# endiqq/Multi-Feature-ViT

Measured on AMD Instinct MI355X. Metric: images/sec (two-stream 224^2 vit_small MF-CA train step), higher is better.
Workload: dtype bf16x3 (split bf16 hi+lo operands, 3 MFMAs per product, f32 accumulate)

## Files before the change

include/mfvit.h:

```cpp
#ifndef MFVIT_H
#define MFVIT_H
#include <stddef.h>
#include <stdint.h>

#ifdef __cplusplus
extern "C" {
#endif

typedef void* mfvit_stream_t;

#define MFVIT_OK 0
#define MFVIT_EINVAL (-22)
#define MFVIT_ENOSYS (-38)
#define MFVIT_ELAUNCH (-5)

#define MFVIT_F32 0
#define MFVIT_BF16 1
#define MFVIT_BF16X3 2
#define MFVIT_F16 3
#define MFVIT_X3F16 4

int mfvit_abi_version(void);
const char* mfvit_build_info(void);

// ... 56 lines not shown
    void* scratch;
} mfvit_vit_attn_req;
size_t mfvit_vit_attn_scratch_bytes(const mfvit_vit_cfg* cfg, const mfvit_vit_attn_req* req);
int mfvit_vit_forward_attn(const mfvit_vit_cfg* cfg, const mfvit_vit_attn_req* req, const float* params, const void* shadow,
                           const float* img, void* workspace, float* features, mfvit_stream_t stream);

typedef struct mfvit_vit_rel_req {
    uint64_t blocks;
    float* maps;
    float* relevance;
    void* scratch;
} mfvit_vit_rel_req;
size_t mfvit_vit_rel_scratch_bytes(const mfvit_vit_cfg* cfg, const mfvit_vit_rel_req* req);
int mfvit_vit_backward_rel(const mfvit_vit_cfg* cfg, const mfvit_vit_rel_req* req, const float* params, const void* shadow, void* workspace,
                           const float* dfeatures, mfvit_stream_t stream);

int mfvit_gpt_forward(const mfvit_vit_cfg* cfg, const float* params, const void* shadow, const float* tokens, void* workspace, float* out,
                      mfvit_stream_t stream);
int mfvit_gpt_backward(const mfvit_vit_cfg* cfg, const float* params, const void* shadow, void* workspace, const float* dout, float* dparams,
                       float* dtokens, mfvit_stream_t stream);

int mfvit_linear_fwd(int dtype, int epilogue, const void* x, int64_t ldx, const void* w, int64_t ldw, const float* bias, void* y,
                     int64_t ldy, void* y2, int64_t ldy2, int M, int N, int K, mfvit_stream_t stream);
int mfvit_linear_dgrad_act(int dtype, const void* dy, int64_t lddy, const void* wt, int64_t ldwt, const void* act_grad, int64_t ldg,
                           void* dx, int64_t lddx, int M, int N, int K, mfvit_stream_t stream);
int mfvit_linear_wgrad(int dtype, const void* dy, int64_t lddy, const void* x, int64_t ldx, float* dw, int64_t lddw, int M, int N, int K,
                       mfvit_stream_t stream);
#define MFVIT_WGRAD_SCRATCH_FLOATS (384 * 128 * 128)
int mfvit_linear_wgrad_ws(int dtype, const void* dy, int64_t lddy, const void* x, int64_t ldx, float* dw, int64_t lddw, int M, int N,
                          int K, float* scratch, mfvit_stream_t stream);
int mfvit_linear_wgrad_pair(int dtype, const void* dy_a, int64_t lddy_a, const void* x_a, int64_t ldx_a, float* dw_a, int64_t lddw_a, float* dbias_a,
                            int Na, const void* dy_b, int64_t lddy_b, const void* x_b, int64_t ldx_b, float* dw_b, int64_t lddw_b, int Nb, int M, int K,
                            mfvit_stream_t stream);
int mfvit_linear_res_ln_fwd(int dtype, const void* a, int64_t lda, const void* w, int64_t ldw, const float* bias, const float* res,
                            int64_t ldres, float* x_out, void* y, int y_f32, const float* gamma, const float* beta, float eps,
                            float* mean, float* rstd, int M, int K, mfvit_stream_t stream);
int mfvit_linear_dgrad_ln_bwd(int dtype, const void* dy, int64_t lddy, const void* wt, int64_t ldwt, const float* x, const float* mean,
                              const float* rstd, const float* gamma, const float* dres, float* dx, void* dx_t, float* dgamma,
                              float* dbeta, float* dcol, int M, int K, mfvit_stream_t stream);
#define MFVIT_ROWP_SCRATCH_FLOATS (264 * 7 * 12 * 512)
int mfvit_linear_res_ln_fwd_ws(int dtype, const void* a, int64_t lda, const void* w, int64_t ldw, const float* bias, const float* res,
                               int64_t ldres, float* x_out, void* y, int y_f32, const float* gamma, const float* beta, float eps,
                               float* mean, float* rstd, int M, int K, float* scratch, mfvit_stream_t stream);
int mfvit_linear_dgrad_ln_bwd_ws(int dtype, const void* dy, int64_t lddy, const void* wt, int64_t ldwt, const float* x, const float* mean,
                                 const float* rstd, const float* gamma, const float* dres, float* dx, void* dx_t, float* dgamma,
                                 float* dbeta, float* dcol, int M, int K, float* scratch, mfvit_stream_t stream);
int mfvit_attention_qkv_dtype(int dtype, int T, int head_dim);
int mfvit_attention_fwd(int dtype, const void* qkv, void* out, float* lse, int B, int T, int H, int head_dim, mfvit_stream_t stream);
int mfvit_attention_bwd(int dtype, const void* qkv, const void* out, const void* dout, const float* lse, void* dqkv, float* dbias_qkv,
                        int B, int T, int H, int head_dim, mfvit_stream_t stream);
int mfvit_attention_drop_fwd(int dtype, const void* qkv, void* out, float* lse, int B, int T, int H, int head_dim, float p, uint64_t seed,
                             uint32_t site, mfvit_stream_t stream);
int mfvit_attention_drop_bwd(int dtype, const void* qkv, const void* out, const void* dout, const float* lse, void* dqkv, int B, int T, int H,
                             int head_dim, float p, uint64_t seed, uint32_t site, mfvit_stream_t stream);
int mfvit_dropout_mask(float p, uint64_t seed, uint32_t site, int64_t n, uint8_t* keep, mfvit_stream_t stream);
int mfvit_layernorm_fwd(int dtype, const float* x, void* y, int y_f32, const float* gamma, const float* beta, float eps, float* mean,
                        float* rstd, int rows, int N, mfvit_stream_t stream);
int mfvit_layernorm_bwd(int dtype, const float* dy, const float* x, const float* mean, const float* rstd, const float* gamma,
                        const float* dres, float* dx, void* dx_t, float* dgamma, float* dbeta, float* dcol, int rows, int N,
                        mfvit_stream_t stream);
int mfvit_cast_transpose(int dtype, const float* src, void* dst, void* dst_t, int R, int C, mfvit_stream_t stream);
int mfvit_head_fwd(const float* x, int64_t ldx, const float* w, const float* b, float* y, int64_t ldy, int M, int N, int K, int accumulate,
                   mfvit_stream_t stream);
int mfvit_head_bwd(const float* dy, int64_t lddy, const float* x, int64_t ldx, const float* w, float* dx, int64_t lddx, int dx_accumulate,
                   float* dw, float* db, int M, int N, int K, mfvit_stream_t stream);
int mfvit_cross_entropy(const float* logits, const int64_t* target, float* loss_mean, float* dlogits, int64_t* preds, int B, int C,
// ... 101 lines not shown
```

multi-feature-vit_amd/csrc/abi_ops.hip:

```cpp
#include "../../include/mfvit.h"
#include "kernels.h"

using namespace mfvit;

extern "C" {

int mfvit_input_transform(const uint8_t* src, const int64_t* desc, const int32_t* tables, int n, int S, int crop, const float* mean3,
                          const float* std3, float* out, mfvit_stream_t stream) {
    if (!src || !desc || !tables || !mean3 || !std3 || !out) return MFVIT_EINVAL;
    if (crop > S) return MFVIT_EINVAL;
    return input_transform(src, (const long long*)desc, tables, n, S, crop, crop, mean3, std3, out, (hipStream_t)stream);
}
int mfvit_input_transform_rect(const uint8_t* src, const int64_t* desc, const int32_t* tables, int n, int S, int out_h, int out_w,
                               const float* mean3, const float* std3, float* out, mfvit_stream_t stream) {
    if (!src || !desc || !tables || !mean3 || !std3 || !out) return MFVIT_EINVAL;
    return input_transform(src, (const long long*)desc, tables, n, S, out_h, out_w, mean3, std3, out, (hipStream_t)stream);
}
size_t mfvit_input_photometric_workspace_bytes(int n, int S) { return input_photometric_workspace_bytes(n, S); }
int mfvit_input_photometric(const uint8_t* src, const int64_t* desc, const int32_t* tables, const int32_t* photo, int n, int S, int max_radius,
                            void* workspace, const float* mean3, const float* std3, float* out, mfvit_stream_t stream) {
    if (!src || !desc || !tables || !photo || !workspace || !mean3 || !std3 || !out) return MFVIT_EINVAL;
    return input_photometric(src, (const long long*)desc, tables, photo, n, S, max_radius, workspace, mean3, std3, out, (hipStream_t)stream);
}
int mfvit_eval_counts(const float* scores, int64_t ld, const int64_t* labels, int n, int C, uint64_t* confusion, int64_t* preds,
// ... 12 lines not shown
    return gemm_nt_tile(dtype, epilogue, p, (hipStream_t)stream);
}
int mfvit_linear_dgrad_act(int dtype, const void* dy, int64_t lddy, const void* wt, int64_t ldwt, const void* act_grad, int64_t ldg,
                           void* dx, int64_t lddx, int M, int N, int K, mfvit_stream_t stream) {
    if (!dy || !wt || !act_grad || !dx) return MFVIT_EINVAL;
    GemmP p = nt(dy, lddy, wt, ldwt, M, N, K);
    p.aux = act_grad; p.ldaux = ldg; p.out0 = dx; p.ldo0 = lddx;
    return gemm_nt_tile(dtype, EPI_GELU_BWD, p, (hipStream_t)stream);
}
int mfvit_linear_wgrad(int dtype, const void* dy, int64_t lddy, const void* x, int64_t ldx, float* dw, int64_t lddw, int M, int N, int K,
                       mfvit_stream_t stream) {
    if (!dy || !x || !dw) return MFVIT_EINVAL;
    GemmP p = nt(dy, lddy, x, ldx, M, N, K);
    p.out0 = dw; p.ldo0 = lddw;
    return gemm_tn(dtype, p, (hipStream_t)stream);
}
int mfvit_linear_wgrad_ws(int dtype, const void* dy, int64_t lddy, const void* x, int64_t ldx, float* dw, int64_t lddw, int M, int N,
                          int K, float* scratch, mfvit_stream_t stream) {
    if (!dy || !x || !dw) return MFVIT_EINVAL;
    GemmP p = nt(dy, lddy, x, ldx, M, N, K);
    p.out0 = dw; p.ldo0 = lddw;
    p.cpart = scratch;
    return gemm_tn(dtype, p, (hipStream_t)stream);
}
int mfvit_linear_wgrad_pair(int dtype, const void* dy_a, int64_t lddy_a, const void* x_a, int64_t ldx_a, float* dw_a, int64_t lddw_a, float* dbias_a,
                            int Na, const void* dy_b, int64_t lddy_b, const void* x_b, int64_t ldx_b, float* dw_b, int64_t lddw_b, int Nb, int M, int K,
                            mfvit_stream_t stream) {
    if (!dy_a || !x_a || !dw_a || !dy_b || !x_b || !dw_b) return MFVIT_EINVAL;
    GemmP a = nt(dy_a, lddy_a, x_a, ldx_a, M, Na, K), b = nt(dy_b, lddy_b, x_b, ldx_b, M, Nb, K);
    a.out0 = dw_a; a.ldo0 = lddw_a; a.cs0 = dbias_a;
    b.out0 = dw_b; b.ldo0 = lddw_b;
    if (!gemm_tn_pair_supported(dtype, a, b)) return MFVIT_ENOSYS;
    return gemm_tn_glds_pair(dtype, a, b, (hipStream_t)stream);
}
int mfvit_linear_res_ln_fwd(int dtype, const void* a, int64_t lda, const void* w, int64_t ldw, const float* bias, const float* res,
                            int64_t ldres, float* x_out, void* y, int y_f32, const float* gamma, const float* beta, float eps,
                            float* mean, float* rstd, int M, int K, mfvit_stream_t stream) {
    return mfvit_linear_res_ln_fwd_ws(dtype, a, lda, w, ldw, bias, res, ldres, x_out, y, y_f32, gamma, beta, eps, mean, rstd, M, K, nullptr, stream);
}
int mfvit_linear_res_ln_fwd_ws(int dtype, const void* a, int64_t lda, const void* w, int64_t ldw, const float* bias, const float* res,
                               int64_t ldres, float* x_out, void* y, int y_f32, const float* gamma, const float* beta, float eps,
                               float* mean, float* rstd, int M, int K, float* scratch, mfvit_stream_t stream) {
    if (!a || !w || !y || !gamma || !beta || ((size_t)scratch & 15)) return MFVIT_EINVAL;
    GemmP p = nt(a, lda, w, ldw, M, 384, K);
    p.kpart = scratch;
    p.bias = bias; p.res = res; p.ldres = ldres;
    p.out0 = x_out; p.ldo0 = 384; p.out1 = y; p.ldo1 = (dtype == MFVIT_BF16X3 && !y_f32) ? 768 : 384; p.y_f32 = y_f32;
    p.gamma = gamma; p.beta = beta; p.eps = eps; p.mean = mean; p.rstd = rstd;
    return gemm_nt_row(dtype, REPI_RES_LN, p, (hipStream_t)stream);
}
int mfvit_linear_dgrad_ln_bwd(int dtype, const void* dy, int64_t lddy, const void* wt, int64_t ldwt, const float* x, const float* mean,
                              const float* rstd, const float* gamma, const float* dres, float* dx, void* dx_t, float* dgamma,
                              float* dbeta, float* dcol, int M, int K, mfvit_stream_t stream) {
    return mfvit_linear_dgrad_ln_bwd_ws(dtype, dy, lddy, wt, ldwt, x, mean, rstd, gamma, dres, dx, dx_t, dgamma, dbeta, dcol, M, K, nullptr, stream);
}
int mfvit_linear_dgrad_ln_bwd_ws(int dtype, const void* dy, int64_t lddy, const void* wt, int64_t ldwt, const float* x, const float* mean,
                                 const float* rstd, const float* gamma, const float* dres, float* dx, void* dx_t, float* dgamma,
                                 float* dbeta, float* dcol, int M, int K, float* scratch, mfvit_stream_t stream) {
    if (!dy || !wt || !x || !mean || !rstd || !gamma || !dx || ((size_t)scratch & 15)) return MFVIT_EINVAL;
    GemmP p = nt(dy, lddy, wt, ldwt, M, 384, K);
    p.kpart = scratch;
    p.aux = x; p.ldaux = 384; p.mean = (float*)mean; p.rstd = (float*)rstd; p.gamma = gamma;
    p.res = dres; p.ldres = 384;
    p.out0 = dx; p.ldo0 = 384; p.out1 = dx_t; p.ldo1 = dtype == MFVIT_BF16X3 ? 768 : 384;
    p.cs0 = dgamma; p.cs1 = dbeta; p.cs2 = dcol;
    return gemm_nt_row(dtype, REPI_LNBWD_RES, p, (hipStream_t)stream);
// ... 62 lines not shown
```

multi-feature-vit_amd/csrc/gemm.cuh:

```cuda
#pragma once
#include "common.cuh"

#include <type_traits>

namespace mfvit {

template <typename T> struct MmaTraits;
template <> struct MmaTraits<bf16> {
    typedef bf16x8 frag_t;
    static constexpr int KSTEP = 16;
    static __device__ __forceinline__ f32x16 mma(frag_t a, frag_t b, f32x16 c) {
        return __builtin_amdgcn_mfma_f32_32x32x16_bf16(a, b, c, 0, 0, 0);
    }
};
template <> struct MmaTraits<sbf16> : MmaTraits<bf16> {};
template <> struct MmaTraits<f16> {
    typedef f16x8 frag_t;
    static constexpr int KSTEP = 16;
    static __device__ __forceinline__ f32x16 mma(frag_t a, frag_t b, f32x16 c) {
        return __builtin_amdgcn_mfma_f32_32x32x16_f16(a, b, c, 0, 0, 0);
    }
};
template <> struct MmaTraits<float> {
    typedef float frag_t;
    static constexpr int KSTEP = 2;
    static __device__ __forceinline__ f32x16 mma(frag_t a, frag_t b, f32x16 c) {
        return __builtin_amdgcn_mfma_f32_32x32x2f32(a, b, c, 0, 0, 0);
    }
};

template <typename T, int R, int BKB> struct KTile;

template <typename T, int R, int BKB> struct KTile16 {
    static constexpr int CPR = BKB / 16;
// ... 120 lines not shown
            const int q = tid + i * NT, m = q / CPRW, c = q % CPRW;
            *(uint4*)(t + ((long)m * Tile::LD + c * EPC) * sizeof(T)) = reg[i];
        }
    }
};

struct GemmP {
    const void* A; long lda;
    const void* W; long ldw;
    int M, N, K;
    const float* bias;
    void* out0; long ldo0;
    void* out1; long ldo1;
    const void* aux; long ldaux;
    const float* res; long ldres;
    const void* res_t; long ldres_t;
    int res_mod, res_off;
    int orow_in, orow_out, orow_off;
    const float* gamma; const float* beta; float eps;
    float* mean; float* rstd;
    float* cs0; float* cs1; float* cs2;
    float* cpart;
    int y_f32;
    int splits;
    float* kpart;
    unsigned* kcnt;
    int rows_per_wg;
    unsigned* omax;
    int omax_rows, omax_hd;
    int nb, nbi;
    long sAo, sAi, sWo, sWi, sOo, sOi, sBo, sBi;
    DropP drop;
    int drop_tpr;
};

template <typename T> __device__ __forceinline__ void apply_batch(GemmP& p, int out_elem_bytes) {
    if (p.nb <= 1) return;
    const int z = blockIdx.z, zo = z / p.nbi, zi = z % p.nbi;
    p.A = (const T*)p.A + zo * p.sAo + zi * p.sAi;
    p.W = (const T*)p.W + zo * p.sWo + zi * p.sWi;
    p.out0 = (char*)p.out0 + (zo * p.sOo + zi * p.sOi) * out_elem_bytes;
    if (p.bias) p.bias += zo * p.sBo + zi * p.sBi;
}

__device__ __forceinline__ int out_row(const GemmP& p, int m) {
    return p.orow_in ? (m / p.orow_in) * p.orow_out + (m % p.orow_in) + p.orow_off : m;
}

__device__ __forceinline__ int acc_row(int reg, int lane) { return (reg & 3) + 8 * (reg >> 2) + 4 * (lane >> 5); }

template <typename T, int BM, int BN, int BKB, int WM, int WN> struct NtLoop {
    static constexpr int NT = WM * WN * 64;
    static constexpr int BK = BKB / (int)sizeof(T);
    static constexpr int TM = BM / WM / 32, TN = BN / WN / 32;
    typedef KTile<T, BM, BKB> TA;
    typedef KTile<T, BN, BKB> TB;
    static constexpr int STAGE_BYTES = TA::BYTES + TB::BYTES;
    static constexpr int LDS_BYTES = 2 * STAGE_BYTES;
    static constexpr bool SPLIT = is_split<T>::value;
    static constexpr bool HALF = SPLIT && BKB == 64;
    static_assert(!SPLIT || BKB == 128 || BKB == 64, "a split K tile is one 32-wide k group ([hi x 32 | lo x 32] = 128 bytes per row) or half of one");

    static __device__ __forceinline__ void compute(const char* ta, const char* tb, int wm, int wn, int lane, f32x16 (&acc)[TM][TN]) {
        if constexpr (HALF) {
            typename MmaTraits<T>::frag_t ah[TM], al[TM], bh[TN], bl[TN];
#pragma unroll
// ... 265 lines not shown
```

multi-feature-vit_amd/csrc/gemm_tn2.hip:

```cpp
#include <stdlib.h>

#include <type_traits>
#include "gemm.cuh"
#include "kernels.h"
#include "prof.h"

namespace mfvit {

namespace {

constexpr int T2_NS = 3;
constexpr int T2_NSP = 4;
constexpr int T2_TILE = 16 * 1024;
constexpr int T2_STAGE = 2 * T2_TILE;

template <typename T> struct T2Geo {
    static constexpr bool SPLIT = is_split<T>::value;
    static constexpr int TW = SPLIT ? 256 : 128;
    static constexpr int KR = SPLIT ? 32 : 64;
    static constexpr int ROWB = TW * 2;
    static constexpr int CPR = ROWB / 16;
    static constexpr int RPI = 64 / CPR;
    static constexpr int NF = TW / 2 / 32;
    static constexpr int BL = 128;
// ... 9 lines not shown
                 : "memory");
}

template <typename T> __device__ __forceinline__ typename Vec8<T>::type t2_frag(const char* t, int rowbase, int s, int lane) {
    constexpr int ROWB = T2Geo<T>::ROWB;
    const int h = lane >> 5, g1 = (lane >> 4) & 1, q = (lane & 15) >> 2, pp = lane & 3;
    const int k0 = 16 * s + 8 * h + q;
    const int col = rowbase + 16 * g1 + 4 * pp;
    const char* a = t + k0 * ROWB + (((col >> 3) ^ (4 * q)) << 4) + (col & 7) * 2;
    typedef __attribute__((address_space(3))) s16x4* lptr;
    const s16x4 lo = __builtin_amdgcn_ds_read_tr16_b64_v4i16((lptr)a);
    const s16x4 hi = __builtin_amdgcn_ds_read_tr16_b64_v4i16((lptr)(a + 4 * ROWB));
    union { struct { s16x4 a, b; } s; typename Vec8<T>::type v; } u;
    u.s.a = lo;
    u.s.b = hi;
    return u.v;
}

template <typename T, bool CS, bool W8, bool IL, bool RM = false>
__global__ __launch_bounds__(W8 ? 512 : 256) void gemm_tn_glds_kernel(GemmP p) {
    typedef T2Geo<T> G;
    constexpr int NWV = W8 ? 8 : 4;
    constexpr int NI = 16 / NWV;
    constexpr int T2_LPS = 2 * NI;
    constexpr bool SPLIT = G::SPLIT;
    constexpr int EP = elems_per<T>::value, TW = G::TW, KR = G::KR, ROWB = G::ROWB, CPR = G::CPR, RPI = G::RPI, NF = G::NF;
    constexpr int NL = 2;
    typedef typename Vec8<T>::type frag_t;
    typedef typename Vec4<T>::elem E16;
    extern __shared__ __attribute__((aligned(16))) char lds[];
    const int tid = threadIdx.x, lane = tid & 63, wave = __builtin_amdgcn_readfirstlane(tid >> 6);
    const int wq = wave & 3, kh = wave >> 2;
    const int wm = wq >> 1, wn = wq & 1;
    const int ntk = p.K * EP / TW;
    const int tiles1 = ntk * (p.N * EP / TW);
    const int tiles = tiles1 + ntk * (p.res_mod * EP / TW);
    const int lin = xcd_remap(blockIdx.x, gridDim.x);
    const int split = lin / tiles, tile_all = lin % tiles;
    const bool second = tile_all >= tiles1;
    const int tile = second ? tile_all - tiles1 : tile_all;
    const int n0 = (tile / ntk) * TW, k0 = (tile % ntk) * TW;
    int chunk = (p.M + p.splits - 1) / p.splits;
    chunk = (chunk + KR - 1) / KR * KR;
    const int mbeg = split * chunk;
    const int mend = min(p.M, mbeg + chunk);
    if (mbeg >= mend) return;
    const int nst = (mend - mbeg + KR - 1) / KR;
    const E16* A = (const E16*)(second ? p.aux : p.A);
    const E16* X = (const E16*)(second ? p.res_t : p.W);
    const long lda_ = second ? p.ldaux : p.lda, ldw_ = second ? p.ldres_t : p.ldw;

    const int lrow = RPI * wave + lane / CPR;
    const int lch = (lane % CPR) ^ (4 * (lrow & 3));
    const unsigned lbase = __builtin_amdgcn_readfirstlane((unsigned)(size_t)(__attribute__((address_space(3))) char*)lds + (unsigned)wave * 1024u);
    auto issue = [&](int st, int slot) {
        const unsigned sa = lbase + (unsigned)slot * T2_STAGE, sb = sa + T2_TILE;
        const int mrow = mbeg + st * KR + lrow;
#pragma unroll
        for (int i = 0; i < NI; ++i) {
            int m = mrow + NWV * RPI * i;
            m = m < p.M ? m : p.M - 1;
            if constexpr (RM) m = out_row(p, m);
            t2_glds16(A + (long)m * lda_ + n0 + lch * 8, sa + i * NWV * 1024);
        }
#pragma unroll
        for (int i = 0; i < NI; ++i) {
            int m = mrow + NWV * RPI * i;
            m = m < p.M ? m : p.M - 1;
            t2_glds16(X + (long)m * ldw_ + k0 + lch * 8, sb + i * NWV * 1024);
        }
    };

    auto dma_one = [&](int st, int slot, int d) __attribute__((always_inline)) {
        const int stc = st < nst ? st : nst - 1;
// ... 229 lines not shown
                        atomicAdd(out + (long)n * ldo_ + k, acc[i][j][r]);
                    }
        }
    }
    if (CS) {
        if (do_cs && (!W8 || kh == 0) && (lane & 31) == 0) {
#pragma unroll
            for (int r = 0; r < 16; ++r) {
                const int n = nw + wn * 32 + acc_row(r, lane);
                if (p.kpart) p.kpart[(long)split * p.N + n] = bacc[0][r];
                else atomicAdd(p.cs0 + n, bacc[0][r]);
            }
        }
    }
}

}

bool gemm_tn_glds_supported(int dtype, const GemmP& p) {
    static int sw_on = INT_MIN;
    if (env_switch("MFVIT_TN_GLDS", 1, sw_on) == 0 || (dtype != MFVIT_BF16 && dtype != MFVIT_BF16X3 && dtype != MFVIT_F16) || p.nb > 1) return false;
    if (p.orow_in && (dtype != MFVIT_BF16X3 || p.cs0 || p.res_mod)) return false;
    if (p.N % 128 || p.K % 128 || p.M < 2048) return false;
    if (p.lda % 8 || p.ldw % 8) return false;
    return true;
}

bool gemm_tn_pair_supported(int dtype, const GemmP& a, const GemmP& b) {
    if (!gemm_tn_glds_supported(dtype, a) || !gemm_tn_glds_supported(dtype, b)) return false;
    if (a.M != b.M || a.K != b.K || b.cs0 || b.cpart || a.splits > 0 || b.splits > 0 || a.res_mod || b.res_mod) return false;
    return true;
}

template <typename T> static int launch_t2(GemmP p, hipStream_t st) {
    typedef T2Geo<T> G;
    const int tiles = ((p.N + p.res_mod) / 128) * (p.K / 128);
    if (p.splits <= 0) {
        const int target = stream_share() >= 2 && p.M < 8192 ? 128 : 256;
        int s = target / tiles;
        const int maxs = (p.M + 4 * G::KR - 1) / (4 * G::KR);
        p.splits = s < 1 ? 1 : (s > maxs ? maxs : s);
    }
    {
        int chunk = (p.M + p.splits - 1) / p.splits;
        chunk = (chunk + G::KR - 1) / G::KR * G::KR;
        p.splits = (p.M + chunk - 1) / chunk;
    }
    if (p.splits < 2 || p.ldo0 % 4 || (p.res_mod && p.ldo1 % 4) || (long)tiles * p.splits > 384) p.cpart = nullptr;
    p.kpart = p.cpart && p.cs0 && (long)tiles * p.splits + 2 <= 384 && p.N % 4 == 0 && (size_t)p.cs0 % 16 == 0 ? p.cpart + (long)p.splits * (p.N + p.res_mod) * p.K : nullptr;
    constexpr int bytes = (is_split<T>::value ? T2_NSP : T2_NS) * T2_STAGE;
    p.rows_per_wg = 0;
    ProfScope ps(PROF_GEMM_TN, 2.0 * p.M * (p.N + p.res_mod) * p.K, 0, st);
    auto go = [&](auto cs, auto w, auto i) {
        constexpr bool CS = decltype(cs)::value, W8 = decltype(w)::value, IL = decltype(i)::value;
        static PerDeviceOnce attr;
        if (attr.first()) {
            (void)hipFuncSetAttribute((const void*)gemm_tn_glds_kernel<T, CS, W8, IL>, hipFuncAttributeMaxDynamicSharedMemorySize, bytes);
        }
        MFVIT_LAUNCH((gemm_tn_glds_kernel<T, CS, W8, IL>), dim3(tiles * p.splits), dim3(W8 ? 512 : 256), bytes, st, p);
    };
    auto go1 = [&](auto cs) { go(cs, std::true_type{}, std::true_type{}); };
    if (p.orow_in) {
        if constexpr (is_split<T>::value) {
            static PerDeviceOnce attr_rm;
            if (attr_rm.first())
                (void)hipFuncSetAttribute((const void*)gemm_tn_glds_kernel<T, false, true, true, true>, hipFuncAttributeMaxDynamicSharedMemorySize, bytes);
            MFVIT_LAUNCH((gemm_tn_glds_kernel<T, false, true, true, true>), dim3(tiles * p.splits), dim3(512), bytes, st, p);
        } else {
            return MFVIT_EINVAL;
        }
    } else if (p.cs0) go1(std::true_type{});
    else go1(std::false_type{});
    MFVIT_CHECK_LAUNCH();
    if (p.cpart) {
        const long stride = (long)(p.N + p.res_mod) * p.K;
        int rc = tn_partial_reduce(p.cpart, p.splits, stride, p.N, p.K, (float*)p.out0, p.ldo0, st);
        if (rc == MFVIT_OK && p.kpart) rc = tn_partial_reduce(p.kpart, p.splits, p.N, 1, p.N, p.cs0, p.N, st);
        if (rc != MFVIT_OK || !p.res_mod) return rc;
        return tn_partial_reduce(p.cpart + (long)p.N * p.K, p.splits, stride, p.res_mod, p.K, (float*)p.out1, p.ldo1, st);
    }
// ... 20 lines not shown
```

multi-feature-vit_amd/csrc/kernels.h:

```cpp
#pragma once
#include "gemm.cuh"

#include <string.h>

namespace mfvit {

enum { EPI_BIAS = 0, EPI_BIAS_GELU = 1, EPI_GELU_BWD = 2, EPI_NONE = 3, EPI_BIAS_RELU = 4,
       EPI_BIAS_X3F16 = 5,
       EPI_BIAS_GELU_DROP = 6,
       EPI_COL2IM16 = 7 };
enum { REPI_RES_LN = 0, REPI_LNBWD_RES = 1,
       REPI_RES_LN_DP = 2 };

int gemm_nt_tile(int dtype, int epi, const GemmP& p, hipStream_t st);
bool gemm_nt_pp_supported(int dtype, int epi, const GemmP& p);
int gemm_nt_pp(int dtype, int epi, const GemmP& p, hipStream_t st);
int gemm_nt_row(int dtype, int repi, const GemmP& p, hipStream_t st);
bool gemm_nt_rowp_supported(int dtype, int repi, const GemmP& p);
int gemm_nt_rowp(int dtype, int repi, const GemmP& p, hipStream_t st);
int input_transform(const unsigned char* src, const long long* desc, const int* tables, int n, int S, int out_h, int out_w,
                    const float* mean, const float* stdv, float* out, hipStream_t st);
int input_transform_u8(const unsigned char* src, const long long* desc, const int* tables, int n, int S, unsigned* frames,
                       hipStream_t st);
size_t input_photometric_workspace_bytes(int n, int S);
int input_photometric(const unsigned char* src, const long long* desc, const int* tables, const int* photo, int n, int S, int max_radius,
                      void* workspace, const float* mean, const float* stdv, float* out, hipStream_t st);
int eval_counts(const float* scores, long ld, const int64_t* labels, int n, int C, unsigned long long* conf, unsigned long long* u2,
                unsigned long long* npos, int64_t* preds, hipStream_t st);
int gemm_tn(int dtype, const GemmP& p, hipStream_t st);
bool gemm_nt_small_supported(int dtype, int epi, const GemmP& p);
int gemm_nt_small(int epi, GemmP p, hipStream_t st);
bool gemm_tn_small_supported(int dtype, const GemmP& p);
int gemm_tn_small(GemmP p, hipStream_t st);
bool gemm_tn_glds_supported(int dtype, const GemmP& p);
int gemm_tn_glds(int dtype, GemmP p, hipStream_t st);
int colpart_reduce(const float* part, int G, int ncols, int nq, float* d0, float* d1, float* d2, hipStream_t st);
struct ColpartJob { const float* part; float* d[3]; int G, ncols, nq; };
struct ColpartBatch { static constexpr int MAXJ = 48; int n; ColpartJob job[MAXJ]; };
ColpartBatch* colpart_batch_begin(ColpartBatch* b);
int colpart_batch_flush(hipStream_t st);
bool gemm_tn_pair_supported(int dtype, const GemmP& a, const GemmP& b);
int gemm_tn_glds_pair(int dtype, GemmP a, const GemmP& b, hipStream_t st);
int tn_partial_reduce(const float* part, int splits, long stride, int N, int K, float* out, long ldo, hipStream_t st);
struct TnPartJob { const float* part; float* out; long stride, ldo; int splits, N, K; long first4; };
struct TnPartBatch { static constexpr int MAXJ = 56; int n; long total4; TnPartJob job[MAXJ]; };
TnPartBatch* tnpart_batch_begin(TnPartBatch* b);
int tnpart_batch_flush(hipStream_t st);

int attn_fwd_exact(int dtype, const void* qkv, void* out, float* lse, int B, int Tn, int H, int HD, hipStream_t st);
int attn_bwd_exact(int dtype, const void* qkv, const void* out, const void* dout, const float* lse, void* dqkv, float* dbias, int B, int Tn,
                   int H, int HD, hipStream_t st);

int attn_qkv_dtype(int dtype, int Tn, int HD);
int attn_fwd(int dtype, const void* qkv, void* out, float* lse, int B, int Tn, int H, int HD, hipStream_t st);
int attn_bwd(int dtype, const void* qkv, const void* out, const void* dout, const float* lse, void* dqkv, float* dbias, int B, int Tn,
             int H, int HD, hipStream_t st, const unsigned* domax = nullptr);

int im2col16(int dtype, const float* img, void* P, int B, int H, int W, hipStream_t st);
int ln_rows(int dtype, int N, const float* in0, long ld0, const float* in1, long ld1, int mod1, float* xout, long ldx, void* y, long ldy,
            int y_f32, const float* gamma, const float* beta, float eps, float* mean, float* rstd, int rows, int row_stride, int row_off,
            int in0_bcast, hipStream_t st);
int ln_bwd_rows(int dtype, int N, const float* dy, long lddy, const float* x, long ldx, const float* mean, const float* rstd,
                const float* gamma, const float* dres, long ldres, float* dx, long lddx, void* dxT, long lddxT, float* dgamma, float* dbeta,
                float* dcol, float* cpart, int rows, int row_stride, int row_off, hipStream_t st, const void* dyT = nullptr, long lddyT = 0);
int add_ln_rows(int dtype, int N, const void* tin, long ldt, const float* pos, long ldp, int pmod, const float* res, long ldres, int rin, int rout,
                int roff, float* xout, long ldx, void* y, long ldy, int y_f32, const float* gamma, const float* beta, float eps, float* mean,
                float* rstd, int rows, hipStream_t st);
int cast_transpose(int dtype, const float* src, void* dst, void* dstT, int R, int C, hipStream_t st);
int cast_transpose_batched(int dtype, const float* src, void* dst, void* dstT, int R, int C, int nb, long s_src, long s_dst, long s_dstT,
                           hipStream_t st);
int linear_small_fwd(const float* x, long ldx, const float* W, const float* b, float* y, long ldy, int M, int N, int K, int accumulate,
                     hipStream_t st);
int linear_small_bwd(const float* dy, long lddy, const float* x, long ldx, const float* W, float* dx, long lddx, int dx_accumulate, float* dW,
                     float* db, int M, int N, int K, hipStream_t st);
int ce_small(const float* logits, const long* target, float* loss_mean, float* dlogits, long* preds, int B, int C, hipStream_t st);
// ... 37 lines not shown
```

multi-feature-vit_amd/mfvit/_lib.py:

```python
import ctypes
import os

import torch
from ctypes import POINTER, Structure, c_char_p, c_double, c_float, c_int, c_int64, c_size_t, c_uint32, c_uint64, c_void_p

_HERE = os.path.dirname(os.path.abspath(__file__))
LIB_PATH = os.environ.get("MFVIT_LIB") or os.path.join(_HERE, "libmfvit_hip.so")
ABI_VERSION = 5

F32, BF16, BF16X3, F16, X3F16 = 0, 1, 2, 3, 4
EPI_BIAS, EPI_BIAS_GELU, EPI_NONE, EPI_BIAS_X3F16 = 0, 1, 3, 5


class VitCfg(Structure):
    _fields_ = [("dtype", c_int), ("batch", c_int), ("img_h", c_int), ("img_w", c_int), ("dim", c_int), ("depth", c_int),
                ("heads", c_int), ("mlp_dim", c_int), ("save_for_backward", c_int), ("stop_grad_conv1", c_int),
                ("ln_eps", c_float), ("token_input", c_int), ("tokens", c_int), ("use_pos", c_int), ("act", c_int),
                ("p_embd", c_float), ("p_attn", c_float), ("p_resid", c_float), ("seed_lo", c_uint32), ("seed_hi", c_uint32),
                ("stream_share", c_int)]


class VitDrop(Structure):
    _fields_ = [("drop", c_float), ("attn_drop", c_float), ("drop_path", POINTER(c_float)), ("seed", c_uint64)]

# ... 16 lines not shown

P = c_void_p
I = c_int
L = c_int64
F = c_float
D = c_double

SIGNATURES = {
    "mfvit_abi_version": (I, []),
    "mfvit_build_info": (c_char_p, []),
    "mfvit_vit_param_count": (c_size_t, [POINTER(VitCfg)]),
    "mfvit_vit_param_layout": (I, [POINTER(VitCfg), POINTER(c_int64)]),
    "mfvit_vit_shadow_bytes": (c_size_t, [POINTER(VitCfg)]),
    "mfvit_vit_prepare_shadow": (I, [POINTER(VitCfg), P, P, P]),
    "mfvit_vit_workspace_bytes": (c_size_t, [POINTER(VitCfg)]),
    "mfvit_vit_forward": (I, [POINTER(VitCfg), P, P, P, P, P, P]),
    "mfvit_vit_backward": (I, [POINTER(VitCfg), P, P, P, P, P, I, I, P]),
    "mfvit_vit_workspace_bytes_drop": (c_size_t, [POINTER(VitCfg), POINTER(VitDrop)]),
    "mfvit_vit_forward_drop": (I, [POINTER(VitCfg), POINTER(VitDrop), P, P, P, P, P, P]),
    "mfvit_vit_backward_drop": (I, [POINTER(VitCfg), POINTER(VitDrop), P, P, P, P, P, I, I, P]),
    "mfvit_vit_workspace_bytes_ex": (c_size_t, [POINTER(VitCfg), POINTER(VitDrop), I]),
    "mfvit_vit_backward_ex": (I, [POINTER(VitCfg), POINTER(VitDrop), P, P, P, P, P, P, I, I, P]),
    "mfvit_vit_attn_scratch_bytes": (c_size_t, [POINTER(VitCfg), POINTER(VitAttnReq)]),
    "mfvit_vit_forward_attn": (I, [POINTER(VitCfg), POINTER(VitAttnReq), P, P, P, P, P, P]),
    "mfvit_vit_rel_scratch_bytes": (c_size_t, [POINTER(VitCfg), POINTER(VitRelReq)]),
    "mfvit_vit_backward_rel": (I, [POINTER(VitCfg), POINTER(VitRelReq), P, P, P, P, P]),
    "mfvit_gpt_forward": (I, [POINTER(VitCfg), P, P, P, P, P, P]),
    "mfvit_gpt_backward": (I, [POINTER(VitCfg), P, P, P, P, P, P, P]),
    "mfvit_linear_fwd": (I, [I, I, P, L, P, L, P, P, L, P, L, I, I, I, P]),
    "mfvit_linear_dgrad_act": (I, [I, P, L, P, L, P, L, P, L, I, I, I, P]),
    "mfvit_linear_wgrad": (I, [I, P, L, P, L, P, L, I, I, I, P]),
    "mfvit_linear_wgrad_ws": (I, [I, P, L, P, L, P, L, I, I, I, P, P]),
    "mfvit_linear_wgrad_pair": (I, [I, P, L, P, L, P, L, P, I, P, L, P, L, P, L, I, I, I, P]),
    "mfvit_linear_res_ln_fwd": (I, [I, P, L, P, L, P, P, L, P, P, I, P, P, F, P, P, I, I, P]),
    "mfvit_linear_dgrad_ln_bwd": (I, [I, P, L, P, L, P, P, P, P, P, P, P, P, P, P, I, I, P]),
    "mfvit_linear_res_ln_fwd_ws": (I, [I, P, L, P, L, P, P, L, P, P, I, P, P, F, P, P, I, I, P, P]),
    "mfvit_linear_dgrad_ln_bwd_ws": (I, [I, P, L, P, L, P, P, P, P, P, P, P, P, P, P, I, I, P, P]),
    "mfvit_attention_fwd": (I, [I, P, P, P, I, I, I, I, P]),
    "mfvit_attention_bwd": (I, [I, P, P, P, P, P, P, I, I, I, I, P]),
    "mfvit_attention_qkv_dtype": (I, [I, I, I]),
    "mfvit_attention_drop_fwd": (I, [I, P, P, P, I, I, I, I, F, c_uint64, c_uint32, P]),
    "mfvit_attention_drop_bwd": (I, [I, P, P, P, P, P, I, I, I, I, F, c_uint64, c_uint32, P]),
    "mfvit_dropout_mask": (I, [F, c_uint64, c_uint32, L, P, P]),
    "mfvit_layernorm_fwd": (I, [I, P, P, I, P, P, F, P, P, I, I, P]),
    "mfvit_layernorm_bwd": (I, [I, P, P, P, P, P, P, P, P, P, P, P, I, I, P]),
    "mfvit_cast_transpose": (I, [I, P, P, P, I, I, P]),
    "mfvit_head_fwd": (I, [P, L, P, P, P, L, I, I, I, I, P]),
    "mfvit_head_bwd": (I, [P, L, P, L, P, P, L, I, P, P, I, I, I, P]),
    "mfvit_cross_entropy": (I, [P, P, P, P, P, I, I, P]),
    "mfvit_cross_entropy_soft": (I, [P, P, P, P, F, P, P, P, I, I, P]),
    "mfvit_batch_mix": (I, [P, P, P, P, P, P, I, I, I, I, P]),
    "mfvit_fusion_param_count": (c_size_t, [POINTER(FusionCfg)]),
    "mfvit_fusion_workspace_bytes": (c_size_t, [POINTER(FusionCfg)]),
    "mfvit_fusion_forward": (I, [POINTER(FusionCfg), P, P, P, P, P, P, P, P, P, P, P, P]),
    "mfvit_fusion_ex_param_count": (c_size_t, [POINTER(FusionCfg), I, I]),
    "mfvit_fusion_ex_workspace_bytes": (c_size_t, [POINTER(FusionCfg), I, I]),
    "mfvit_fusion_ex_forward": (I, [POINTER(FusionCfg), I, I, P, P, P, P, P, P, P, P, P, P, P, P]),
    "mfvit_fusion_ex_backward": (I, [POINTER(FusionCfg), I, I, P, P, P, P, P, P, P, P, P, P, P, P, P, P, P, P, P]),
    "mfvit_bn_stats": (I, [I, P, I, I, P, P, P]),
    "mfvit_bn_combine": (I, [P, P, P, I, I, F, F, P, P, P, P, P]),
    "mfvit_bn_apply": (I, [I, P, P, P, P, P, I, P, I, I, P]),
    "mfvit_bn_bwd_sums": (I, [I, P, P, P, P, P, I, I, I, P, P, P]),
    "mfvit_bn_bwd_apply": (I, [I, P, P, P, P, P, P, I, P, P, F, P, I, I, P]),
    "mfvit_l2norm_fwd": (I, [P, P, P, I, I, F, P]),
    "mfvit_l2norm_bwd": (I, [P, P, P, P, I, I, P]),
    "mfvit_rowdot": (I, [P, P, P, L, F, I, I, P]),
# ... 104 lines not shown
```

multi-feature-vit_amd/mfvit/ops.py:

```python
import torch

from . import _lib
from ._lib import BF16, BF16X3, EPI_BIAS, EPI_BIAS_GELU, EPI_BIAS_X3F16, EPI_NONE, F16, F32, X3F16, check, lib, ptr, require_cuda, stream

_TORCH_OF = {BF16: torch.bfloat16, BF16X3: torch.bfloat16, F16: torch.float16, F32: torch.float32}


def _tdtype(code):
    return _TORCH_OF[code]


def _code_of(t, split=False):
    if t.dtype == torch.bfloat16:
        return BF16X3 if split else BF16
    if t.dtype == torch.float16 and not split:
        return F16
    if t.dtype == torch.float32 and not split:
        return F32
    raise _lib.MfvitError(f"unsupported dtype {t.dtype}{' for a split tensor' if split else ''}")


def split_pack(x):
    x = x.float()
    hi = x.to(torch.bfloat16)
# ... 59 lines not shown
WGRAD_SCRATCH_FLOATS = 384 * 128 * 128


_wgrad_scratch = {}


def wgrad_scratch(device):
    key = (device.index, torch.cuda.current_stream(device).cuda_stream)
    t = _wgrad_scratch.get(key)
    if t is None:
        t = _wgrad_scratch[key] = torch.empty(WGRAD_SCRATCH_FLOATS, device=device, dtype=torch.float32)
    return t


def linear_wgrad(dy, x, out=None, scratch=None, split=False):
    require_cuda(dy, x)
    code = _code_of(dy, split)
    e = 2 if split else 1
    M, N = dy.shape[0], dy.shape[1] // e
    K = x.shape[1] // e
    if out is None:
        out = torch.zeros(N, K, device=dy.device, dtype=torch.float32)
    if scratch is not None:
        if scratch.dtype != torch.float32 or scratch.numel() < WGRAD_SCRATCH_FLOATS:
            raise _lib.MfvitError("wgrad scratch must be float32 with at least WGRAD_SCRATCH_FLOATS elements")
        check(lib().mfvit_linear_wgrad_ws(code, ptr(dy), dy.stride(0), ptr(x), x.stride(0), ptr(out), out.stride(0), M, N, K,
                                          ptr(scratch), stream()), "mfvit_linear_wgrad_ws")
    else:
        check(lib().mfvit_linear_wgrad(code, ptr(dy), dy.stride(0), ptr(x), x.stride(0), ptr(out), out.stride(0), M, N, K, stream()),
              "mfvit_linear_wgrad")
    return out


def linear_wgrad_pair(dy_a, x_a, dy_b, x_b, want_dbias=True, split=False):
    require_cuda(dy_a, x_a, dy_b, x_b)
    code = _code_of(dy_a, split)
    e = 2 if split else 1
    M, Na, Nb = dy_a.shape[0], dy_a.shape[1] // e, dy_b.shape[1] // e
    K = x_a.shape[1] // e
    if dy_b.shape[0] != M or x_a.shape[0] != M or x_b.shape[0] != M or x_b.shape[1] // e != K:
        raise _lib.MfvitError("linear_wgrad_pair: the two GEMMs must share M and K")
    dw_a = torch.zeros(Na, K, device=dy_a.device, dtype=torch.float32)
    dw_b = torch.zeros(Nb, K, device=dy_a.device, dtype=torch.float32)
    db_a = torch.zeros(Na, device=dy_a.device, dtype=torch.float32) if want_dbias else None
    check(lib().mfvit_linear_wgrad_pair(code, ptr(dy_a), dy_a.stride(0), ptr(x_a), x_a.stride(0), ptr(dw_a), dw_a.stride(0), ptr(db_a), Na,
                                        ptr(dy_b), dy_b.stride(0), ptr(x_b), x_b.stride(0), ptr(dw_b), dw_b.stride(0), Nb, M, K, stream()),
          "mfvit_linear_wgrad_pair")
    return dw_a, db_a, dw_b


ROWP_SCRATCH_FLOATS = 264 * 7 * 12 * 512


def linear_res_ln_fwd(a, w, bias, res, gamma, beta, eps, y_f32=False, split=False, scratch=None):
    require_cuda(a, w, res)
    code = _code_of(a, split)
    e = 2 if split else 1
    M, K = a.shape[0], a.shape[1] // e
    x_out = torch.empty(M, 384, device=a.device, dtype=torch.float32)
    y = torch.empty(M, 384 if y_f32 else 384 * e, device=a.device, dtype=torch.float32 if y_f32 else a.dtype)
    mean = torch.empty(M, device=a.device, dtype=torch.float32)
    rstd = torch.empty_like(mean)
    check(lib().mfvit_linear_res_ln_fwd_ws(code, ptr(a), a.stride(0), ptr(w), w.stride(0), ptr(bias), ptr(res),
                                           res.stride(0) if res is not None else 0, ptr(x_out), ptr(y), int(y_f32), ptr(gamma),
                                           ptr(beta), eps, ptr(mean), ptr(rstd), M, K, ptr(scratch), stream()), "mfvit_linear_res_ln_fwd_ws")
    return x_out, y, mean, rstd


def linear_dgrad_ln_bwd(dy, wt, x, mean, rstd, gamma, dres, want_copy=True, split=False, scratch=None):
    require_cuda(dy, wt, x)
    code = _code_of(dy, split)
    e = 2 if split else 1
    M, K = dy.shape[0], dy.shape[1] // e
    dx = torch.empty(M, 384, device=dy.device, dtype=torch.float32)
    dx_t = torch.empty(M, 384 * e, device=dy.device, dtype=dy.dtype) if want_copy else None
    dgamma = torch.zeros(384, device=dy.device, dtype=torch.float32)
    dbeta = torch.zeros_like(dgamma)
    dcol = torch.zeros_like(dgamma)
    check(lib().mfvit_linear_dgrad_ln_bwd_ws(code, ptr(dy), dy.stride(0), ptr(wt), wt.stride(0), ptr(x), ptr(mean), ptr(rstd),
                                             ptr(gamma), ptr(dres), ptr(dx), ptr(dx_t), ptr(dgamma), ptr(dbeta), ptr(dcol), M, K,
                                             ptr(scratch), stream()), "mfvit_linear_dgrad_ln_bwd_ws")
# ... 185 lines not shown
```

Baseline: 5037.

## Pick wgrad tile traversal order by modeled per-XCD cache traffic

```diff
diff --git a/include/mfvit.h b/include/mfvit.h
--- a/include/mfvit.h
+++ b/include/mfvit.h
@@ -112,6 +112,10 @@
 int mfvit_linear_wgrad_pair(int dtype, const void* dy_a, int64_t lddy_a, const void* x_a, int64_t ldx_a, float* dw_a, int64_t lddw_a, float* dbias_a,
                             int Na, const void* dy_b, int64_t lddy_b, const void* x_b, int64_t ldx_b, float* dw_b, int64_t lddw_b, int Nb, int M, int K,
                             mfvit_stream_t stream);
+int mfvit_linear_wgrad_pair_ws(int dtype, const void* dy_a, int64_t lddy_a, const void* x_a, int64_t ldx_a, float* dw_a, int64_t lddw_a, float* dbias_a,
+                               int Na, const void* dy_b, int64_t lddy_b, const void* x_b, int64_t ldx_b, float* dw_b, int64_t lddw_b, int Nb, int M, int K,
+                               float* scratch, mfvit_stream_t stream);
+int mfvit_wgrad_tile_order(int dtype, int M, int Na, int Nb, int K, int order, double* model_bytes);
 int mfvit_linear_res_ln_fwd(int dtype, const void* a, int64_t lda, const void* w, int64_t ldw, const float* bias, const float* res,
                             int64_t ldres, float* x_out, void* y, int y_f32, const float* gamma, const float* beta, float eps,
                             float* mean, float* rstd, int M, int K, mfvit_stream_t stream);
diff --git a/multi-feature-vit_amd/csrc/abi_ops.hip b/multi-feature-vit_amd/csrc/abi_ops.hip
--- a/multi-feature-vit_amd/csrc/abi_ops.hip
+++ b/multi-feature-vit_amd/csrc/abi_ops.hip
@@ -68,6 +68,20 @@
     b.out0 = dw_b; b.ldo0 = lddw_b;
     if (!gemm_tn_pair_supported(dtype, a, b)) return MFVIT_ENOSYS;
     return gemm_tn_glds_pair(dtype, a, b, (hipStream_t)stream);
+}
+int mfvit_linear_wgrad_pair_ws(int dtype, const void* dy_a, int64_t lddy_a, const void* x_a, int64_t ldx_a, float* dw_a, int64_t lddw_a, float* dbias_a,
+                               int Na, const void* dy_b, int64_t lddy_b, const void* x_b, int64_t ldx_b, float* dw_b, int64_t lddw_b, int Nb, int M, int K,
+                               float* scratch, mfvit_stream_t stream) {
+    if (!dy_a || !x_a || !dw_a || !dy_b || !x_b || !dw_b) return MFVIT_EINVAL;
+    GemmP a = nt(dy_a, lddy_a, x_a, ldx_a, M, Na, K), b = nt(dy_b, lddy_b, x_b, ldx_b, M, Nb, K);
+    a.out0 = dw_a; a.ldo0 = lddw_a; a.cs0 = dbias_a;
+    a.cpart = scratch;
+    b.out0 = dw_b; b.ldo0 = lddw_b;
+    if (!gemm_tn_pair_supported(dtype, a, b)) return MFVIT_ENOSYS;
+    return gemm_tn_glds_pair(dtype, a, b, (hipStream_t)stream);
+}
+int mfvit_wgrad_tile_order(int dtype, int M, int Na, int Nb, int K, int order, double* model_bytes) {
+    return gemm_tn_glds_order(dtype, M, Na, Nb, K, order, model_bytes);
 }
 int mfvit_linear_res_ln_fwd(int dtype, const void* a, int64_t lda, const void* w, int64_t ldw, const float* bias, const float* res,
                             int64_t ldres, float* x_out, void* y, int y_f32, const float* gamma, const float* beta, float eps,
diff --git a/multi-feature-vit_amd/csrc/gemm.cuh b/multi-feature-vit_amd/csrc/gemm.cuh
--- a/multi-feature-vit_amd/csrc/gemm.cuh
+++ b/multi-feature-vit_amd/csrc/gemm.cuh
@@ -1,5 +1,6 @@
 #pragma once
 #include "common.cuh"
+#include "tn_order.h"
 
 #include <type_traits>
 
@@ -186,6 +187,7 @@
     long sAo, sAi, sWo, sWi, sOo, sOi, sBo, sBi;
     DropP drop;
     int drop_tpr;
+    int tn_order;
 };
 
 template <typename T> __device__ __forceinline__ void apply_batch(GemmP& p, int out_elem_bytes) {
diff --git a/multi-feature-vit_amd/csrc/gemm_tn2.hip b/multi-feature-vit_amd/csrc/gemm_tn2.hip
--- a/multi-feature-vit_amd/csrc/gemm_tn2.hip
+++ b/multi-feature-vit_amd/csrc/gemm_tn2.hip
@@ -65,14 +65,10 @@
     const int tid = threadIdx.x, lane = tid & 63, wave = __builtin_amdgcn_readfirstlane(tid >> 6);
     const int wq = wave & 3, kh = wave >> 2;
     const int wm = wq >> 1, wn = wq & 1;
-    const int ntk = p.K * EP / TW;
-    const int tiles1 = ntk * (p.N * EP / TW);
-    const int tiles = tiles1 + ntk * (p.res_mod * EP / TW);
-    const int lin = xcd_remap(blockIdx.x, gridDim.x);
-    const int split = lin / tiles, tile_all = lin % tiles;
-    const bool second = tile_all >= tiles1;
-    const int tile = second ? tile_all - tiles1 : tile_all;
-    const int n0 = (tile / ntk) * TW, k0 = (tile % ntk) * TW;
+    const TnTile tt = tn_decode(tn_xcd_lin(blockIdx.x, gridDim.x), p.N * EP / TW, p.res_mod * EP / TW, p.K * EP / TW, p.tn_order);
+    const int split = tt.split;
+    const bool second = tt.second;
+    const int n0 = tt.n * TW, k0 = tt.k * TW;
     int chunk = (p.M + p.splits - 1) / p.splits;
     chunk = (chunk + KR - 1) / KR * KR;
     const int mbeg = split * chunk;
@@ -368,20 +364,50 @@
     return true;
 }
 
+static int tn_order_switch() {
+    static int cache = INT_MIN;
+    static const bool live = [] { const char* e = getenv("MFVIT_AB_LIVE"); return e && e[0] == '1'; }();
+    if (cache == INT_MIN || live) {
+        const char* e = getenv("MFVIT_TN_ORDER");
+        cache = e && e[0] >= '0' && e[0] <= '3' && !e[1] ? e[0] - '0' : -1;
+    }
+    return cache;
+}
+
+static int t2_order(int M, int N1, int N2, int K, int splits, int KR, int elem_bytes) {
+    const int forced = tn_order_switch();
+    if (forced >= 0) return forced & (N2 > 0 ? 3 : 1);
+    struct Key { int M, N1, N2, K, splits, KR, eb, order; };
+    static thread_local Key cache[8];
+    static thread_local int cache_n = 0, cache_next = 0;
+    for (int i = 0; i < cache_n; ++i) {
+        const Key& c = cache[i];
+        if (c.M == M && c.N1 == N1 && c.N2 == N2 && c.K == K && c.splits == splits && c.KR == KR && c.eb == elem_bytes) return c.order;
+    }
+    const int order = tn_pick_order(M, N1, N2, K, splits, KR, elem_bytes);
+    cache[cache_next] = Key{M, N1, N2, K, splits, KR, elem_bytes, order};
+    cache_next = (cache_next + 1) & 7;
+    if (cache_n < 8) ++cache_n;
+    return order;
+}
+
+int gemm_tn_glds_order(int dtype, int M, int N1, int N2, int K, int order, double* bytes_out) {
+    if (dtype != MFVIT_BF16 && dtype != MFVIT_BF16X3 && dtype != MFVIT_F16) return MFVIT_EINVAL;
+    if (M < 1 || N1 < 128 || N1 % 128 || N2 < 0 || N2 % 128 || K < 128 || K % 128 || order > 3) return MFVIT_EINVAL;
+    const bool split = dtype == MFVIT_BF16X3;
+    const int KR = split ? T2Geo<sbf16>::KR : T2Geo<bf16>::KR, eb = split ? 4 : 2;
+    const int splits = tn_plan_splits(M, ((N1 + N2) / 128) * (K / 128), KR, stream_share() >= 2 && M < 8192 ? 128 : 256, 0);
+    if (order < 0) order = tn_pick_order(M, N1, N2, K, splits, KR, eb);
+    order &= N2 > 0 ? 3 : 1;
+    if (bytes_out) *bytes_out = tn_order_bytes(M, N1, N2, K, splits, KR, eb, order);
+    return order;
+}
+
 template <typename T> static int launch_t2(GemmP p, hipStream_t st) {
     typedef T2Geo<T> G;
     const int tiles = ((p.N + p.res_mod) / 128) * (p.K / 128);
-    if (p.splits <= 0) {
-        const int target = stream_share() >= 2 && p.M < 8192 ? 128 : 256;
-        int s = target / tiles;
-        const int maxs = (p.M + 4 * G::KR - 1) / (4 * G::KR);
-        p.splits = s < 1 ? 1 : (s > maxs ? maxs : s);
-    }
-    {
-        int chunk = (p.M + p.splits - 1) / p.splits;
-        chunk = (chunk + G::KR - 1) / G::KR * G::KR;
-        p.splits = (p.M + chunk - 1) / chunk;
-    }
+    p.splits = tn_plan_splits(p.M, tiles, G::KR, stream_share() >= 2 && p.M < 8192 ? 128 : 256, p.splits);
+    p.tn_order = t2_order(p.M, p.N, p.res_mod, p.K, p.splits, G::KR, is_split<T>::value ? 4 : 2);
     if (p.splits < 2 || p.ldo0 % 4 || (p.res_mod && p.ldo1 % 4) || (long)tiles * p.splits > 384) p.cpart = nullptr;
     p.kpart = p.cpart && p.cs0 && (long)tiles * p.splits + 2 <= 384 && p.N % 4 == 0 && (size_t)p.cs0 % 16 == 0 ? p.cpart + (long)p.splits * (p.N + p.res_mod) * p.K : nullptr;
     constexpr int bytes = (is_split<T>::value ? T2_NSP : T2_NS) * T2_STAGE;
diff --git a/multi-feature-vit_amd/csrc/kernels.h b/multi-feature-vit_amd/csrc/kernels.h
--- a/multi-feature-vit_amd/csrc/kernels.h
+++ b/multi-feature-vit_amd/csrc/kernels.h
@@ -41,6 +41,7 @@
 int colpart_batch_flush(hipStream_t st);
 bool gemm_tn_pair_supported(int dtype, const GemmP& a, const GemmP& b);
 int gemm_tn_glds_pair(int dtype, GemmP a, const GemmP& b, hipStream_t st);
+int gemm_tn_glds_order(int dtype, int M, int N1, int N2, int K, int order, double* bytes_out);
 int tn_partial_reduce(const float* part, int splits, long stride, int N, int K, float* out, long ldo, hipStream_t st);
 struct TnPartJob { const float* part; float* out; long stride, ldo; int splits, N, K; long first4; };
 struct TnPartBatch { static constexpr int MAXJ = 56; int n; long total4; TnPartJob job[MAXJ]; };
diff --git a/multi-feature-vit_amd/csrc/tn_order.h b/multi-feature-vit_amd/csrc/tn_order.h
--- /dev/null
+++ b/multi-feature-vit_amd/csrc/tn_order.h
@@ -0,0 +1,82 @@
+#pragma once
+
+#if defined(__HIPCC__)
+#define MFVIT_TN_HD __host__ __device__ __forceinline__
+#else
+#define MFVIT_TN_HD inline
+#endif
+
+namespace mfvit {
+
+MFVIT_TN_HD int tn_xcd_lin(int bid, int nwg) {
+    const int q = nwg >> 3, r = nwg & 7, xcd = bid & 7, loc = bid >> 3;
+    const int base = xcd < r ? xcd * (q + 1) : r * (q + 1) + (xcd - r) * q;
+    return base + loc;
+}
+
+struct TnTile { int split, second, n, k; };
+
+MFVIT_TN_HD TnTile tn_decode(int lin, int ntn1, int ntn2, int ntk, int order) {
+    const int tiles1 = ntk * ntn1, tiles = tiles1 + ntk * ntn2;
+    TnTile t;
+    t.split = lin / tiles;
+    const int tile_all = lin - t.split * tiles;
+    t.second = tile_all >= tiles1;
+    const int tile = t.second ? tile_all - tiles1 : tile_all;
+    const bool nfast = (order >> t.second) & 1;
+    const int inner = nfast ? (t.second ? ntn2 : ntn1) : ntk;
+    const int hi = tile / inner, lo = tile - hi * inner;
+    t.n = nfast ? lo : hi;
+    t.k = nfast ? hi : lo;
+    return t;
+}
+
+inline int tn_plan_splits(int M, int tiles, int KR, int target, int forced) {
+    int splits = forced;
+    if (splits <= 0) {
+        const int s = target / tiles, maxs = (M + 4 * KR - 1) / (4 * KR);
+        splits = s < 1 ? 1 : (s > maxs ? maxs : s);
+    }
+    int chunk = (M + splits - 1) / splits;
+    chunk = (chunk + KR - 1) / KR * KR;
+    return (M + chunk - 1) / chunk;
+}
+
+inline double tn_order_bytes(int M, int N1, int N2, int K, int splits, int KR, int elem_bytes, int order) {
+    const int ntn1 = N1 / 128, ntn2 = N2 / 128, ntk = K / 128;
+    const int tiles = (ntn1 + ntn2) * ntk, nwg = tiles * splits;
+    const int maxn = ntn1 > ntn2 ? ntn1 : ntn2, slices = maxn > ntk ? maxn : ntk;
+    if (nwg <= 0 || splits > 1024 || slices > 1024) return -1.0;
+    int chunk = (M + splits - 1) / splits;
+    chunk = (chunk + KR - 1) / KR * KR;
+    double bytes = 0.0;
+    const int nkey = splits * 4;
+    unsigned char* seen = new unsigned char[(long)nkey * slices];
+    for (int xcd = 0; xcd < 8; ++xcd) {
+        for (long i = 0; i < (long)nkey * slices; ++i) seen[i] = 0;
+        for (int bid = xcd; bid < nwg; bid += 8) {
+            const TnTile t = tn_decode(tn_xcd_lin(bid, nwg), ntn1, ntn2, ntk, order);
+            const int mbeg = t.split * chunk, mend = M < mbeg + chunk ? M : mbeg + chunk;
+            const double item = (double)(mend > mbeg ? mend - mbeg : 0) * 128.0 * elem_bytes;
+            unsigned char& a = seen[(long)((t.split * 2 + t.second) * 2 + 0) * slices + t.n];
+            unsigned char& x = seen[(long)((t.split * 2 + t.second) * 2 + 1) * slices + t.k];
+            if (!a) { a = 1; bytes += item; }
+            if (!x) { x = 1; bytes += item; }
+        }
+    }
+    delete[] seen;
+    return bytes;
+}
+
+inline int tn_pick_order(int M, int N1, int N2, int K, int splits, int KR, int elem_bytes) {
+    const int ncand = N2 > 0 ? 4 : 2;
+    int best = 0;
+    double best_b = tn_order_bytes(M, N1, N2, K, splits, KR, elem_bytes, 0);
+    for (int o = 1; o < ncand; ++o) {
+        const double b = tn_order_bytes(M, N1, N2, K, splits, KR, elem_bytes, o);
+        if (b >= 0.0 && b < best_b) { best = o; best_b = b; }
+    }
+    return best;
+}
+
+}
diff --git a/multi-feature-vit_amd/mfvit/_lib.py b/multi-feature-vit_amd/mfvit/_lib.py
--- a/multi-feature-vit_amd/mfvit/_lib.py
+++ b/multi-feature-vit_amd/mfvit/_lib.py
@@ -72,6 +72,8 @@
     "mfvit_linear_wgrad": (I, [I, P, L, P, L, P, L, I, I, I, P]),
     "mfvit_linear_wgrad_ws": (I, [I, P, L, P, L, P, L, I, I, I, P, P]),
     "mfvit_linear_wgrad_pair": (I, [I, P, L, P, L, P, L, P, I, P, L, P, L, P, L, I, I, I, P]),
+    "mfvit_linear_wgrad_pair_ws": (I, [I, P, L, P, L, P, L, P, I, P, L, P, L, P, L, I, I, I, P, P]),
+    "mfvit_wgrad_tile_order": (I, [I, I, I, I, I, I, POINTER(c_double)]),
     "mfvit_linear_res_ln_fwd": (I, [I, P, L, P, L, P, P, L, P, P, I, P, P, F, P, P, I, I, P]),
     "mfvit_linear_dgrad_ln_bwd": (I, [I, P, L, P, L, P, P, P, P, P, P, P, P, P, P, I, I, P]),
     "mfvit_linear_res_ln_fwd_ws": (I, [I, P, L, P, L, P, P, L, P, P, I, P, P, F, P, P, I, I, P, P]),
diff --git a/multi-feature-vit_amd/mfvit/ops.py b/multi-feature-vit_amd/mfvit/ops.py
--- a/multi-feature-vit_amd/mfvit/ops.py
+++ b/multi-feature-vit_amd/mfvit/ops.py
@@ -115,7 +115,7 @@
     return out
 
 
-def linear_wgrad_pair(dy_a, x_a, dy_b, x_b, want_dbias=True, split=False):
+def linear_wgrad_pair(dy_a, x_a, dy_b, x_b, want_dbias=True, split=False, scratch=None):
     require_cuda(dy_a, x_a, dy_b, x_b)
     code = _code_of(dy_a, split)
     e = 2 if split else 1
@@ -126,10 +126,25 @@
     dw_a = torch.zeros(Na, K, device=dy_a.device, dtype=torch.float32)
     dw_b = torch.zeros(Nb, K, device=dy_a.device, dtype=torch.float32)
     db_a = torch.zeros(Na, device=dy_a.device, dtype=torch.float32) if want_dbias else None
+    if scratch is not None:
+        if scratch.dtype != torch.float32 or scratch.numel() < WGRAD_SCRATCH_FLOATS:
+            raise _lib.MfvitError("wgrad scratch must be float32 with at least WGRAD_SCRATCH_FLOATS elements")
+        check(lib().mfvit_linear_wgrad_pair_ws(code, ptr(dy_a), dy_a.stride(0), ptr(x_a), x_a.stride(0), ptr(dw_a), dw_a.stride(0), ptr(db_a), Na,
+                                               ptr(dy_b), dy_b.stride(0), ptr(x_b), x_b.stride(0), ptr(dw_b), dw_b.stride(0), Nb, M, K, ptr(scratch),
+                                               stream()), "mfvit_linear_wgrad_pair_ws")
+        return dw_a, db_a, dw_b
     check(lib().mfvit_linear_wgrad_pair(code, ptr(dy_a), dy_a.stride(0), ptr(x_a), x_a.stride(0), ptr(dw_a), dw_a.stride(0), ptr(db_a), Na,
                                         ptr(dy_b), dy_b.stride(0), ptr(x_b), x_b.stride(0), ptr(dw_b), dw_b.stride(0), Nb, M, K, stream()),
           "mfvit_linear_wgrad_pair")
     return dw_a, db_a, dw_b
+
+
+def wgrad_tile_order(M, N, K, N2=0, order=None, precision="bf16x3"):
+    import ctypes
+    b = ctypes.c_double(0.0)
+    o = lib().mfvit_wgrad_tile_order(_lib.dtype_code(precision), M, N, N2, K, -1 if order is None else order, ctypes.byref(b))
+    check(min(o, 0), "mfvit_wgrad_tile_order")
+    return o, b.value
 
 
 ROWP_SCRATCH_FLOATS = 264 * 7 * 12 * 512
```

Result: no change. 5052, median of 6 (+0.3%).
